# cbalint13/opencv-dlco

Hardware: AMD Instinct MI355X
Metric: pj-learn patch-pairs/sec (higher is better)
Workload: dtype f32; 1 GPU; pj-learn configs[1] Liberty-shaped, rank ~64: 500000 pair-rows x PR-dim 8192, batch 200+200 per GPU (global 200+200), mu=0.0025 gamma=0.5, fp32, rank 48 after 3893 steps; device= (gfx950:sramecc+:xnack-), burn_in_steps=300

## Files before the change

include/dlco.h:

```cpp
#ifndef DLCO_H
#define DLCO_H

#include <stddef.h>
#include <stdint.h>

#ifdef __cplusplus
extern "C" {
#endif

#define DLCO_OK            0
#define DLCO_ERR_INVALID  -2
#define DLCO_ERR_HIP      -3
#define DLCO_ERR_NODEVICE -4
#define DLCO_ERR_NOCONV   -5
#define DLCO_ERR_COMM     -6

typedef struct dlco_ctx dlco_ctx;

typedef struct dlco_cfg {
    int32_t  F;
    int32_t  N;
    int32_t  B;
    float    mu;
    float    gamma;
// ... 51 lines not shown
typedef int (*dlco_allgather_fn)(void *user, int32_t which, size_t bytes_per_rank);
int dlco_set_allgather(dlco_ctx *ctx, dlco_allgather_fn fn, void *user);
int dlco_comm_unique_id(void *out_id, size_t cap, const char *rccl_path);
int dlco_comm_init(dlco_ctx *ctx, const void *id, size_t id_bytes, const char *rccl_path);
int dlco_comm_init_host(dlco_ctx *ctx, const char *shm_name);
int dlco_comm_destroy(dlco_ctx *ctx);
int dlco_stream(dlco_ctx *ctx, void **stream);
int dlco_sync(dlco_ctx *ctx);

int dlco_get_batch(const dlco_ctx *ctx, int32_t *pos_rows, int32_t *neg_rows,
                   float *pos_dist, float *neg_dist, int32_t *rho, int32_t *kappa);

int dlco_get_t(const dlco_ctx *ctx, uint32_t *t);
int dlco_get_W(dlco_ctx *ctx, float *W_host , int32_t *r);
int dlco_get_A(dlco_ctx *ctx, float *A_host );
int dlco_get_dfavg(dlco_ctx *ctx, float *dfavg_host );
int dlco_set_state(dlco_ctx *ctx, uint32_t t, const float *dfavg_host, const float *W_host, int32_t r);

int dlco_validate(dlco_ctx *ctx, float *loss_val, float *regul, int32_t *rank);

int dlco_stats(dlco_ctx *ctx, const float *W_host, int32_t r, int32_t *dim, float *fpr95, double *auc);

int dlco_project_sqdist(dlco_ctx *ctx, const int32_t *row_ids_host, int32_t n,
                        const float *W_host, int32_t r, float *out_host);
int dlco_viol_counts(dlco_ctx *ctx, const float *pd_host, const float *nd_host, int32_t B,
                     int32_t *rho_host, int32_t *kappa_host);
int dlco_grad_rda(dlco_ctx *ctx, const int32_t *pos_rows_host, const int32_t *neg_rows_host,
                  const int32_t *rho_host, const int32_t *kappa_host, int32_t B,
                  float alpha, float beta, const float *dfavg_in_host, float *dfavg_out_host);
int dlco_psd_project(dlco_ctx *ctx, const float *dfavg_host, uint32_t t,
                     float *W_host, int32_t *r, float *A_host );
int dlco_sym_product(dlco_ctx *ctx, const float *X_host, int32_t rows, const float *G_host, int32_t mode,
                     float *out_host);
int dlco_hinge_sum(dlco_ctx *ctx, const float *pos_host, int32_t n_pos,
                   const float *neg_host, int32_t n_neg, double *out);
int dlco_roc_stats(dlco_ctx *ctx, const float *dist_host, const uint8_t *labels_host, int32_t n,
                   float *fpr95, double *auc);

typedef struct dlco_log_entry {
    uint32_t t;
    int32_t  is_best;
    int32_t  saved;
    float    loss_val, regul, obj, obj_best;
    int32_t  rank, rank_best;
    int32_t  dim;
    double   auc, auc_best;
    float    fpr95, fpr95_best;
    double   vtime;
    int32_t  nonconv;
    int32_t  reserved;
} dlco_log_entry;
int dlco_log_step(dlco_ctx *ctx, dlco_log_entry *out);
int dlco_get_saved(dlco_ctx *ctx, float *W_host, int32_t *r, float *A_host);

int dlco_profile_enable(dlco_ctx *ctx, int32_t on);
int dlco_profile_read(dlco_ctx *ctx, const char *kernel, int64_t *launches, double *total_ms);
int dlco_counters(const dlco_ctx *ctx, int64_t out[8]);
int dlco_eig_stats(const dlco_ctx *ctx, int64_t *iters, int64_t *product_rows, int64_t *jacobi_sweeps,
                   int32_t *block_rows);

typedef struct dlco_pr_ctx dlco_pr_ctx;
const char *dlco_pr_last_error(const dlco_pr_ctx *ctx);
int dlco_pr_create(dlco_pr_ctx **out, int32_t F, int32_t N, float mu, float gamma, uint64_t seed, int32_t device);
void dlco_pr_destroy(dlco_pr_ctx *ctx);
int dlco_pr_device_name(const dlco_pr_ctx *ctx, char *buf, size_t cap, int *cc_major, int *cc_minor);
int dlco_pr_set_data(dlco_pr_ctx *ctx, const float *dists_host, const uint8_t *labels_host);
// ... 98 lines not shown
```

opencv-dlco_amd/__init__.py:

```python
import ctypes as C
import os
import subprocess

import numpy as np

_HERE = os.path.dirname(os.path.abspath(__file__))
LIB_PATH = os.path.join(_HERE, "libdlco.so")
HEADER_PATH = os.path.join(os.path.dirname(_HERE), "include", "dlco.h")

OK, ERR_INVALID, ERR_HIP, ERR_NODEVICE, ERR_NOCONV, ERR_COMM = 0, -2, -3, -4, -5, -6
BUF_DIST, BUF_GRAD, BUF_DFAVG, BUF_W, BUF_GATHER, BUF_DATA = 1, 2, 3, 4, 5, 6
ALLGATHER_FN = C.CFUNCTYPE(C.c_int, C.c_void_p, C.c_int32, C.c_size_t)
DETECT_THRESHOLD = 100 * 100 * 256 * 256


class DlcoError(RuntimeError):
    def __init__(self, code, msg):
        super().__init__("libdlco error %d: %s" % (code, msg))
        self.code = code


class Cfg(C.Structure):
    _fields_ = [
        ("F", C.c_int32), ("N", C.c_int32), ("B", C.c_int32),
        ("mu", C.c_float), ("gamma", C.c_float),
        ("seed", C.c_uint64),
        ("device", C.c_int32), ("rank", C.c_int32), ("world", C.c_int32),
        ("eig_tol", C.c_float), ("eig_guard", C.c_int32), ("eig_max_iter", C.c_int32),
        ("shard", C.c_int32), ("strict_conv", C.c_int32), ("grad_bf16", C.c_int32),
        ("reserved", C.c_int32 * 5),
    ]


class LogEntry(C.Structure):
    _fields_ = [
        ("t", C.c_uint32), ("is_best", C.c_int32), ("saved", C.c_int32),
        ("loss_val", C.c_float), ("regul", C.c_float), ("obj", C.c_float), ("obj_best", C.c_float),
        ("rank", C.c_int32), ("rank_best", C.c_int32), ("dim", C.c_int32),
        ("auc", C.c_double), ("auc_best", C.c_double),
        ("fpr95", C.c_float), ("fpr95_best", C.c_float),
        ("vtime", C.c_double),
        ("nonconv", C.c_int32), ("reserved", C.c_int32),
    ]


def build(verbose=False):
    cmd = ["make", "-C", os.path.join(_HERE, "csrc"), "-j8"]
    if not verbose:
        cmd.insert(1, "-s")
    subprocess.check_call(cmd)


_lib = None
f32p, i32p, u8p = C.POINTER(C.c_float), C.POINTER(C.c_int32), C.POINTER(C.c_uint8)


def load():
    global _lib
    if _lib is not None:
        return _lib
    if not os.path.exists(LIB_PATH):
        raise DlcoError(ERR_NODEVICE, "%s is missing: run __graft_entry__.build() (no CPU fallback exists)" % LIB_PATH)
    L = C.CDLL(LIB_PATH)
    vp = C.c_void_p
    L.dlco_version.restype = C.c_char_p
    L.dlco_last_error.restype = C.c_char_p
    L.dlco_last_error.argtypes = [vp]
    L.dlco_cfg_default.argtypes = [C.POINTER(Cfg)]
    L.dlco_cfg_default.restype = None
    L.dlco_ctx_create.argtypes = [C.POINTER(vp), C.POINTER(Cfg)]
    L.dlco_ctx_destroy.argtypes = [vp]
    L.dlco_ctx_destroy.restype = None
    L.dlco_device_name.argtypes = [vp, C.c_char_p, C.c_size_t, C.POINTER(C.c_int), C.POINTER(C.c_int)]
    L.dlco_set_data.argtypes = [vp, f32p, u8p]
    L.dlco_set_data_device.argtypes = [vp, vp, u8p]
    L.dlco_set_data_shared.argtypes = [vp, vp]
    L.dlco_device_width.argtypes = [vp]
    L.dlco_set_pairs.argtypes = [vp, f32p, C.c_int32, i32p]
    L.dlco_synth_data.argtypes = [vp, f32p, C.c_int32, C.c_uint64, C.c_float, C.c_float, C.c_float, C.c_float]
    L.dlco_get_rows.argtypes = [vp, C.c_int32, C.c_int32, f32p]
    L.dlco_get_index.argtypes = [vp, i32p, i32p, i32p, i32p, i32p, i32p]
    for name in ("dlco_step", "dlco_step_begin", "dlco_step_grad", "dlco_step_finish", "dlco_sync"):
        getattr(L, name).argtypes = [vp]
    L.dlco_steps.argtypes = [vp, C.c_int32]
    L.dlco_dev_buffer.argtypes = [vp, C.c_int32, C.POINTER(vp), C.POINTER(C.c_size_t)]
    L.dlco_bind_buffer.argtypes = [vp, C.c_int32, vp, C.c_size_t]
    L.dlco_stream.argtypes = [vp, C.POINTER(vp)]
    L.dlco_set_allgather.argtypes = [vp, ALLGATHER_FN, vp]
    L.dlco_comm_unique_id.argtypes = [vp, C.c_size_t, C.c_char_p]
    L.dlco_comm_init.argtypes = [vp, vp, C.c_size_t, C.c_char_p]
    L.dlco_comm_destroy.argtypes = [vp]
    L.dlco_get_batch.argtypes = [vp, i32p, i32p, f32p, f32p, i32p, i32p]
    L.dlco_get_t.argtypes = [vp, C.POINTER(C.c_uint32)]
    L.dlco_get_W.argtypes = [vp, f32p, i32p]
    L.dlco_get_A.argtypes = [vp, f32p]
    L.dlco_get_dfavg.argtypes = [vp, f32p]
    L.dlco_set_state.argtypes = [vp, C.c_uint32, f32p, f32p, C.c_int32]
    L.dlco_validate.argtypes = [vp, f32p, f32p, i32p]
    L.dlco_stats.argtypes = [vp, f32p, C.c_int32, i32p, f32p, C.POINTER(C.c_double)]
    L.dlco_project_sqdist.argtypes = [vp, i32p, C.c_int32, f32p, C.c_int32, f32p]
    L.dlco_viol_counts.argtypes = [vp, f32p, f32p, C.c_int32, i32p, i32p]
    L.dlco_grad_rda.argtypes = [vp, i32p, i32p, i32p, i32p, C.c_int32, C.c_float, C.c_float, f32p, f32p]
    L.dlco_psd_project.argtypes = [vp, f32p, C.c_uint32, f32p, i32p, f32p]
    L.dlco_hinge_sum.argtypes = [vp, f32p, C.c_int32, f32p, C.c_int32, C.POINTER(C.c_double)]
    L.dlco_sym_product.argtypes = [vp, f32p, C.c_int32, f32p, C.c_int32, f32p]
    L.dlco_roc_stats.argtypes = [vp, f32p, u8p, C.c_int32, f32p, C.POINTER(C.c_double)]
    L.dlco_log_step.argtypes = [vp, C.POINTER(LogEntry)]
    L.dlco_get_saved.argtypes = [vp, f32p, i32p, f32p]
    L.dlco_profile_enable.argtypes = [vp, C.c_int32]
    L.dlco_profile_read.argtypes = [vp, C.c_char_p, C.POINTER(C.c_int64), C.POINTER(C.c_double)]
    L.dlco_eig_stats.argtypes = [vp, C.POINTER(C.c_int64), C.POINTER(C.c_int64), C.POINTER(C.c_int64), i32p]
    L.dlco_counters.argtypes = [vp, C.POINTER(C.c_int64)]
    i64 = C.c_int64
    L.dlco_set_pairs_device.argtypes = [vp, vp, C.c_int32, i32p]
    L.dlco_desc_last_error.restype = C.c_char_p
    L.dlco_desc_last_error.argtypes = [vp]
    L.dlco_desc_create.argtypes = [C.POINTER(vp), C.c_float, C.c_int32, C.c_int32, C.c_int32]
    L.dlco_desc_destroy.argtypes = [vp]
    L.dlco_desc_destroy.restype = None
    L.dlco_desc_select_filters.argtypes = [f32p, C.c_int32, C.c_int32, f32p, C.c_int32, f32p, C.POINTER(C.c_int32)]
    L.dlco_desc_set_filters.argtypes = [vp, f32p, C.c_int32]
    L.dlco_desc_size.argtypes = [vp]
    L.dlco_desc_size.restype = C.c_int32
    L.dlco_desc_transform.argtypes = [vp, u8p, f32p]
    L.dlco_desc_compute.argtypes = [vp, u8p, i64, f32p]
    L.dlco_desc_compute_device.argtypes = [vp, u8p, i64, vp, i64]
    L.dlco_desc_pair_dists.argtypes = [vp, u8p, i64, i32p, i64, f32p, u8p]
    L.dlco_desc_full_dists.argtypes = [vp, u8p, i64, i32p, i64, f32p, u8p]
    L.dlco_desc_set_projection.argtypes = [vp, f32p, C.c_int32, C.c_int32]
    L.dlco_desc_projected_size.argtypes = [vp]
    L.dlco_desc_projected_size.restype = C.c_int32
    L.dlco_desc_describe.argtypes = [vp, u8p, i64, f32p]
    L.dlco_desc_describe_device.argtypes = [vp, u8p, i64, vp, i64]
    L.dlco_desc_set_image.argtypes = [vp, u8p, C.c_int32, C.c_int32, i64]
    L.dlco_desc_set_image_device.argtypes = [vp, vp, C.c_int32, C.c_int32, i64]
    L.dlco_desc_extract_patches.argtypes = [vp, f32p, i64, C.c_float, C.c_int32, u8p, u8p]
    L.dlco_desc_describe_keypoints.argtypes = [vp, f32p, i64, C.c_float, C.c_int32, f32p, u8p]
    L.dlco_desc_describe_keypoints_device.argtypes = [vp, f32p, i64, C.c_float, C.c_int32, vp, i64, u8p]
# ... 277 lines not shown
    def project_sqdist(self, row_ids, W):
        ids, w = _i32(row_ids), _f32(W)
        out = np.empty(ids.size, np.float32)
        self._ck(self.L.dlco_project_sqdist(self.h, _p(ids, i32p), ids.size, _p(w, f32p), w.shape[0] if w.size else 0, _p(out, f32p)))
        return out

    def viol_counts(self, pd, nd):
        pd, nd = _f32(pd), _f32(nd)
        rho, kap = np.empty(pd.size, np.int32), np.empty(pd.size, np.int32)
        self._ck(self.L.dlco_viol_counts(self.h, _p(pd, f32p), _p(nd, f32p), pd.size, _p(rho, i32p), _p(kap, i32p)))
        return rho, kap

    def grad_rda(self, pos_rows, neg_rows, rho, kappa, alpha, beta, dfavg_in=None):
        pr, nr, rho, kap = _i32(pos_rows), _i32(neg_rows), _i32(rho), _i32(kappa)
        d = None if dfavg_in is None else _f32(dfavg_in)
        out = np.empty((self.F, self.F), np.float32)
        self._ck(self.L.dlco_grad_rda(self.h, _p(pr, i32p), _p(nr, i32p), _p(rho, i32p), _p(kap, i32p), pr.size, alpha, beta, _p(d, f32p), _p(out, f32p)))
        return out

    def psd_project(self, dfavg, t, want_A=True):
        d = _f32(dfavg)
        W = np.empty((self.F, self.F), np.float32)
        A = np.empty((self.F, self.F), np.float32) if want_A else None
        r = C.c_int32()
        self._ck(self.L.dlco_psd_project(self.h, _p(d, f32p), t, _p(W, f32p), C.byref(r), _p(A, f32p)))
        return W[:r.value].copy(), A

    def sym_product(self, X, G, mode=0):
        x, g = _f32(X), _f32(G)
        out = np.empty_like(x)
        self._ck(self.L.dlco_sym_product(self.h, _p(x, f32p), x.shape[0], _p(g, f32p), mode, _p(out, f32p)))
        return out

    def hinge_sum(self, pos, neg):
        p, n = _f32(pos), _f32(neg)
        out = C.c_double()
        self._ck(self.L.dlco_hinge_sum(self.h, _p(p, f32p), p.size, _p(n, f32p), n.size, C.byref(out)))
        return out.value

    def roc_stats(self, dist, labels):
        d, l = _f32(dist), np.ascontiguousarray(labels, np.uint8).ravel()
        f, a = C.c_float(), C.c_double()
        self._ck(self.L.dlco_roc_stats(self.h, _p(d, f32p), _p(l, u8p), d.size, C.byref(f), C.byref(a)))
        return f.value, a.value

    def profile_enable(self, on=True):
        self._ck(self.L.dlco_profile_enable(self.h, int(on)))

    def profile_read(self, kernel="grad_syrk"):
        n, ms = C.c_int64(), C.c_double()
        self._ck(self.L.dlco_profile_read(self.h, kernel.encode(), C.byref(n), C.byref(ms)))
        return n.value, ms.value

    def counters(self):
        out = (C.c_int64 * 8)()
        self._ck(self.L.dlco_counters(self.h, out))
        return dict(steps=out[0], active_rows=out[1], nonconverged=out[2], jacobi_barrier_timeouts=out[3],
                    rank_update_passes=out[4], rank_update_check=out[5] * 1e-9, locked_passes=out[6], locked_rows=out[7])

    def eig_stats(self):
        a, b, c_, d = C.c_int64(), C.c_int64(), C.c_int64(), C.c_int32()
        self._ck(self.L.dlco_eig_stats(self.h, C.byref(a), C.byref(b), C.byref(c_), C.byref(d)))
        return dict(iters=a.value, product_rows=b.value, jacobi_sweeps=c_.value, block_rows=d.value)


class PrContext:
# ... 411 lines not shown
```

opencv-dlco_amd/csrc/dlco_api.cpp:

```cpp
#include "../../include/dlco.h"

#include "dlco_internal.hpp"
#include "eig_tracker.hpp"
#include "pair_index.hpp"
#include "rccl_comm.hpp"
#include "host_comm.hpp"

#include <algorithm>
#include <cfloat>
#include <chrono>
#include <cmath>
#include <cstring>

using namespace dlco;

static thread_local std::string g_last_error;

namespace {
struct EnvSwitch { const char *name, *purpose; };
const EnvSwitch kEnvSwitches[] = {
    {"DLCO_SYRK_FP32", "gradient SYRK as the k-ordered fp32 MFMA chain (syrk_rda_kernel8) instead of split-bf16 planes"},
    {"DLCO_NO_PACKED", "full F x F dual average where the packed upper-tile form would apply"},
    {"DLCO_FORCE_SHARD", "column-sharded layout (cfg.shard) on a single rank: the multi-GPU path on one GPU"},
    {"DLCO_NO_RANK_UPDATE", "first filter term from a product with the dual average, not from the step's rank update"},
// ... 1109 lines not shown
            ok = skinny_product_sym(X.p, F, rows, Gp.p, F, 1.0f, out.p, F, nullptr, 0.f, nullptr, 0.f, hi.p, lo.p, slab.p, c->stream,
                                    mode == 4 ? lo2.p : nullptr);
            sync(c);
        } else if (mode == 1 || mode == 2) {
            DevBuf<char> hi, lo, lo2;
            hi.alloc(bf16x2_plane_bytes(rows, F)); lo.alloc(bf16x2_plane_bytes(rows, F));
            if (mode == 2) lo2.alloc(bf16x2_plane_bytes(rows, F));
            DevBuf<float> slab;
            slab.alloc(bf16x2_slab_floats(rows, F));
            ok = skinny_product_bf16x2(X.p, F, rows, G.p, F, F, F, 1.0f, out.p, F, nullptr, 0.f, nullptr, 0.f, hi.p, lo.p, slab.p,
                                       c->stream, 0, mode == 2 ? lo2.p : nullptr);
            sync(c);
        } else {
            GemmArgs g;
            g.M = rows; g.N = F; g.K = F;
            g.A.p = X.p; g.A.ld = F; g.A.kmajor = false;
            g.B.p = G.p; g.B.ld = F; g.B.kmajor = true;
            g.C = out.p; g.ldc = F;
            const int bm = rows <= 64 ? 64 : 128;
            const long tiles = (long)((rows + bm - 1) / bm) * ((F + 127) / 128);
            g.split_k = split_k_slices(tiles, 1024, F, 256);
            DevBuf<float> slab;
            slab.alloc(gemm_slab_floats(rows, F, g.split_k));
            g.slab = slab.p;
            gemm_f32(g, c->stream);
            sync(c);
            ok = true;
        }
        DLCO_CHECK(ok, DLCO_ERR_INVALID, "dlco_sym_product: shape not supported by this mode");
        d2h_rows(c, out_host, out.p, (size_t)rows);
    });
}

int dlco_hinge_sum(dlco_ctx *c, const float *pos_host, int32_t n_pos, const float *neg_host, int32_t n_neg, double *out)
{
    if (!c || !out || n_pos < 0 || n_neg < 0) return DLCO_ERR_INVALID;
    return guarded(c, [&] {
        DLCO_HIP(hipSetDevice(c->cfg.device));
        *out = 0.0;
        if (n_pos == 0) return;
        DevBuf<float> p, n, rows;
        p.alloc(n_pos); n.alloc(std::max(n_neg, 1)); rows.alloc(n_pos);
        h2d(c, p.p, pos_host, (size_t)n_pos * sizeof(float));
        if (n_neg) h2d(c, n.p, neg_host, (size_t)n_neg * sizeof(float));
        hinge_rows(p.p, n_pos, n.p, n_neg, rows.p, c->stream);
        sum_f32_to_f64(rows.p, n_pos, c->dscal.p, c->stream);
        d2h(c, out, c->dscal.p, sizeof(double));
    });
}

int dlco_roc_stats(dlco_ctx *c, const float *dist_host, const uint8_t *labels_host, int32_t n, float *fpr95, double *auc)
{
    if (!c || !dist_host || !labels_host || !fpr95 || !auc || n < 1) return DLCO_ERR_INVALID;
    return guarded(c, [&] {
        DLCO_HIP(hipSetDevice(c->cfg.device));
        DevBuf<float> d; DevBuf<uint8_t> l;
        d.alloc(n); l.alloc(n);
        h2d(c, d.p, dist_host, (size_t)n * sizeof(float));
        h2d(c, l.p, labels_host, (size_t)n);
        RocWork *w = roc_work_create(n);
        try { roc_stats(w, d.p, l.p, n, fpr95, auc, c->stream); } catch (...) { roc_work_destroy(w); throw; }
        roc_work_destroy(w);
    });
}

int dlco_log_step(dlco_ctx *c, dlco_log_entry *out)
// ... 110 lines not shown
```

opencv-dlco_amd/csrc/dlco_internal.hpp:

```cpp
#pragma once

#include "../../include/dlco.h"
#include "match_slices.hpp"

#include <hip/hip_runtime.h>

#include <algorithm>
#include <climits>
#include <cstdint>
#include <cstdio>
#include <cstdlib>
#include <cstring>
#include <functional>
#include <mutex>
#include <utility>
#include <stdexcept>
#include <string>
#include <type_traits>
#include <vector>

namespace patch_rules { struct Frame; }

namespace dlco {

// ... 121 lines not shown
        r.used = 0;
    }
    void drain_all() { for (int i = 0; i < PROF_SLOTS; i++) drain(i); }
    void reset() { drain_all(); for (auto &r : rec) { r.ms = 0.0; r.n = 0; } }
};

struct GemmOperand {
    const float *p = nullptr;
    long ld = 0;
    bool kmajor = false;
    const int32_t *row_ids = nullptr;
    const int32_t *row_ids2 = nullptr;
    const float *row_scale = nullptr;
};

struct GemmArgs {
    int M = 0, N = 0, K = 0;
    GemmOperand A, B;
    float *C = nullptr;
    long ldc = 0;
    float alpha = 1.0f, beta = 0.0f;
    const float *E1 = nullptr;
    float b1 = 0.0f;
    const float *E2 = nullptr;
    float b2 = 0.0f;
    const int *k_dev = nullptr;
    int split_k = 1;
    float *slab = nullptr;
    bool upper_only = false;
    const float *B2 = nullptr;
    float *C2 = nullptr;
    bool small_m_tiles = false;
    bool small_n_tiles = false;
};

void gemm_f32(const GemmArgs &a, hipStream_t s);
size_t bf16x2_plane_bytes(int M, int K);
size_t bf16x2_slab_floats(int M, int N, int ksplit = 0);
void split_planes_bf16(const float *X, long ldx, int M, int K, void *hi, void *lo, void *lo2, hipStream_t s);
bool skinny_product_bf16x2(const float *X, long ldx, int M, const float *G, long ldg, int N, int K, float alpha, float *C,
                           long ldc, const float *E1, float b1, const float *E2, float b2, void *plane_hi, void *plane_lo,
                           float *slab, hipStream_t s, int ksplit = 0, void *plane_lo2 = nullptr, bool g_tiled = false);
size_t project_rows_plane_bytes(int K);
bool project_rows_sqdist(const float *W, long ldw, int r, const float *D, long ldd, int F, const int32_t *ids, const int32_t *ids2,
                         long row0, int nrows, float *dist, void *plane_hi, void *plane_lo, void *plane_lo2, bool bf16, hipStream_t s);
bool project_rows_slab(const float *W, long ldw, int r, const float *D, long ldd, int F, const int32_t *ids, const int32_t *ids2,
                       int nrows, int ksplit, float *slab, long ldn, void *plane_hi, void *plane_lo, void *plane_lo2, bool bf16,
                       hipStream_t s);
struct RankCoeffJob {
    const float *proj = nullptr;
    long ldp = 0;
    int nw = 0, m = 0, MT = 0;
    const float *wscale = nullptr;
    const int32_t *slot = nullptr;
    void *frag = nullptr;
};
void syrk_mirror_upper(float *C, long ldc, int F, hipStream_t s);
size_t syrk_planes_bytes(int kmax, int F);
bool syrk_rda_f32(const float *D, long ldd, const int32_t *ids, const int32_t *ids2, const float *w, const int *k_dev,
                  int kmax, int F, float alpha, float beta, float *C, long ldc, hipStream_t s, int slab_col0 = 0,
                  int slab_cols = 0, bool bf16 = false, bool packed = false, void *planes_ws = nullptr,
                  const RankCoeffJob *coeff_job = nullptr);
int syrk_planes_mode(bool bf16);
size_t rank_coeff_bytes(int m, int kmax);
bool rank_first_term(const float *Y, const float *Q, long ld, int m, int F, float ay, float aq, float ac, float *out,
                     const float *proj, long ldp, int nw, const float *wscale, const int32_t *slot, const float *w,
                     const int *k_dev, int kmax, const void *planes, void *coeff_ws, void *plane_hi, void *plane_lo, hipStream_t s,
                     bool coeff_ready = false, int planes_mode = 3);
size_t syrk_packed_floats(int F);
// ... 115 lines not shown
```

opencv-dlco_amd/csrc/kernels_gemm.hip:

```cpp
#include "dlco_internal.hpp"

namespace dlco {

typedef float f32x16 __attribute__((ext_vector_type(16)));
typedef float f32x4 __attribute__((ext_vector_type(4)));

namespace {

constexpr int BK = 16;
constexpr int PAD = 4;
constexpr int NT = 256;

struct OperandDev {
    const float *p;
    long ld;
    const int32_t *row_ids;
    const float *row_scale;
    int vec_ok;
    const int32_t *row_ids2;
};

__device__ __forceinline__ f32x4 load4(const float *src, int pos, int limit, int vec_ok)
{
    f32x4 v = {0.f, 0.f, 0.f, 0.f};
    if (vec_ok && pos + 3 < limit) {
        v = *reinterpret_cast<const f32x4 *>(src);
    } else {
        v[0] = src[0];
        if (pos + 1 < limit) v[1] = src[1];
        if (pos + 2 < limit) v[2] = src[2];
        if (pos + 3 < limit) v[3] = src[3];
    }
    return v;
}

struct GemmDev {
    int M, N, K;
    OperandDev A, B;
    float *C;
    long ldc;
    float alpha, beta, b1, b2;
    const float *E1, *E2;
    const int *k_dev;
    int k_chunk;
// ... 7 lines not shown
__device__ __forceinline__ void load_tile(const OperandDev &op, int t0, int tmax, int k0, int kend,
                                          f32x4 (&regs)[BT / 64])
{
    const int tid = threadIdx.x;
#pragma unroll
    for (int u = 0; u < BT / 64; u++) {
        const int f = tid + NT * u;
        f32x4 v = {0.f, 0.f, 0.f, 0.f};
        if (KM) {
            const int row = f / (BT / 4), c4 = f % (BT / 4);
            const int k = k0 + row, col = t0 + c4 * 4;
            if (k < kend && col < tmax) {
                const long mr = op.row_ids ? (long)op.row_ids[k] : (long)k;
                v = load4(op.p + mr * op.ld + col, col, tmax, op.vec_ok);
                if (op.row_ids2) v -= load4(op.p + (long)op.row_ids2[k] * op.ld + col, col, tmax, op.vec_ok);
                if (op.row_scale) {
                    const float sc = op.row_scale[k];
                    v *= sc;
                }
            }
        } else {
            const int row = f / (BK / 4), kq = f % (BK / 4);
            const int t = t0 + row, k = k0 + kq * 4;
            if (t < tmax && k < kend) {
                const long mr = op.row_ids ? (long)op.row_ids[t] : (long)t;
                v = load4(op.p + mr * op.ld + k, k, kend, op.vec_ok);
                if (op.row_ids2) v -= load4(op.p + (long)op.row_ids2[t] * op.ld + k, k, kend, op.vec_ok);
            }
        }
        regs[u] = v;
    }
}

template <int BT, bool KM>
__device__ __forceinline__ void store_tile(float (*lds)[BT + PAD], const f32x4 (&regs)[BT / 64])
{
    const int tid = threadIdx.x;
#pragma unroll
    for (int u = 0; u < BT / 64; u++) {
        const int f = tid + NT * u;
        if (KM) {
            const int row = f / (BT / 4), c4 = f % (BT / 4);
            *reinterpret_cast<f32x4 *>(&lds[row][c4 * 4]) = regs[u];
        } else {
            const int row = f / (BK / 4), kq = f % (BK / 4);
            lds[kq * 4 + 0][row] = regs[u][0];
            lds[kq * 4 + 1][row] = regs[u][1];
            lds[kq * 4 + 2][row] = regs[u][2];
            lds[kq * 4 + 3][row] = regs[u][3];
        }
    }
}

template <int WM, int WN, bool A_KM, bool B_KM>
__global__ __launch_bounds__(NT) void gemm_kernel(GemmDev g)
{
    constexpr int BM = 64 * WM, BN = 64 * WN;
    __shared__ __attribute__((aligned(16))) float As[2][BK][BM + PAD];
    __shared__ __attribute__((aligned(16))) float Bs[2][BK][BN + PAD];

    const int bi = blockIdx.y, bj = blockIdx.x;
    if (g.upper_only && bj * BN + BN <= bi * BM) return;
    const int i0 = bi * BM, j0 = bj * BN;
    const int lane = threadIdx.x & 63, wave = threadIdx.x >> 6;
    const int wm = wave >> 1, wn = wave & 1;

    int kz = blockIdx.z;
    if (g.B2) {
        if (kz == 1) { g.B.p = g.B2; g.C = g.C2; }
        kz = 0;
    }
    int kbeg = kz * g.k_chunk;
    int kend = min(g.K, kbeg + g.k_chunk);
    if (g.k_dev) kend = min(kend, *g.k_dev);

    f32x16 acc[WM][WN];
#pragma unroll
    for (int a = 0; a < WM; a++)
#pragma unroll
        for (int b = 0; b < WN; b++)
#pragma unroll
            for (int r = 0; r < 16; r++) acc[a][b][r] = 0.f;

    const int nk = kend > kbeg ? (kend - kbeg + BK - 1) / BK : 0;
    f32x4 ra[BM / 64], rb[BN / 64];
    if (nk > 0) {
        load_tile<BM, A_KM>(g.A, i0, g.M, kbeg, kend, ra);
        load_tile<BN, B_KM>(g.B, j0, g.N, kbeg, kend, rb);
        store_tile<BM, A_KM>(As[0], ra);
        store_tile<BN, B_KM>(Bs[0], rb);
    }
    __syncthreads();
    for (int kt = 0; kt < nk; kt++) {
        const int buf = kt & 1;
        if (kt + 1 < nk) {
            load_tile<BM, A_KM>(g.A, i0, g.M, kbeg + (kt + 1) * BK, kend, ra);
            load_tile<BN, B_KM>(g.B, j0, g.N, kbeg + (kt + 1) * BK, kend, rb);
        }
        const int lr = lane & 31, lk = lane >> 5;
#pragma unroll
        for (int kk = 0; kk < BK / 2; kk++) {
            float af[WM], bf[WN];
#pragma unroll
            for (int a = 0; a < WM; a++) af[a] = As[buf][2 * kk + lk][wm * 32 * WM + a * 32 + lr];
#pragma unroll
            for (int b = 0; b < WN; b++) bf[b] = Bs[buf][2 * kk + lk][wn * 32 * WN + b * 32 + lr];
#pragma unroll
            for (int a = 0; a < WM; a++)
#pragma unroll
                for (int b = 0; b < WN; b++)
                    acc[a][b] = __builtin_amdgcn_mfma_f32_32x32x2f32(af[a], bf[b], acc[a][b], 0, 0, 0);
        }
        if (kt + 1 < nk) {
            store_tile<BM, A_KM>(As[buf ^ 1], ra);
            store_tile<BN, B_KM>(Bs[buf ^ 1], rb);
        }
        __syncthreads();
    }

    const int lc = lane & 31, lh = lane >> 5;
#pragma unroll
    for (int a = 0; a < WM; a++)
#pragma unroll
        for (int b = 0; b < WN; b++)
#pragma unroll
            for (int r = 0; r < 16; r++) {
                const int i = i0 + wm * 32 * WM + a * 32 + (r & 3) + 8 * (r >> 2) + 4 * lh;
                const int j = j0 + wn * 32 * WN + b * 32 + lc;
                if (i >= g.M || j >= g.N) continue;
                if (g.slab) {
                    g.slab[((long)blockIdx.z * g.M + i) * g.N + j] = acc[a][b][r];
                    continue;
                }
                if (g.upper_only && j < i) continue;
                const long idx = (long)i * g.ldc + j;
                float o = g.alpha * acc[a][b][r];
                if (g.beta != 0.f) o += g.beta * g.C[idx];
                if (g.E1) o += g.b1 * g.E1[idx];
                if (g.E2) o += g.b2 * g.E2[idx];
                g.C[idx] = o;
                if (g.upper_only && j > i) g.C[(long)j * g.ldc + i] = o;
            }
}

__global__ void splitk_reduce_kernel(const float *slab, int split, int M, int N, float *C, long ldc, float alpha,
                                     float beta, const float *E1, float b1, const float *E2, float b2)
{
    const long total = (long)M * N;
    const int zl = threadIdx.x & 15;
    for (long e = ((long)blockIdx.x * blockDim.x + threadIdx.x) >> 4; e < total; e += ((long)gridDim.x * blockDim.x) >> 4) {
// ... 3 lines not shown
        s += __int_as_float(__builtin_amdgcn_update_dpp(0, __float_as_int(s), 0xB1, 0xF, 0xF, true));
        s += __int_as_float(__builtin_amdgcn_update_dpp(0, __float_as_int(s), 0x4E, 0xF, 0xF, true));
        s += __int_as_float(__builtin_amdgcn_update_dpp(0, __float_as_int(s), 0x141, 0xF, 0xF, true));
        s += __int_as_float(__builtin_amdgcn_update_dpp(0, __float_as_int(s), 0x140, 0xF, 0xF, true));
        if (zl != 0) continue;
        const long idx = (long)i * ldc + j;
        float o = alpha * s;
        if (beta != 0.f) o += beta * C[idx];
        if (E1) o += b1 * E1[idx];
        if (E2) o += b2 * E2[idx];
        C[idx] = o;
    }
}

__global__ __launch_bounds__(256) void splitk_reduce_wide_kernel(const float *slab, int split, int M, int N, float *C,
                                                                 long ldc, float alpha, float beta, const float *E1,
                                                                 float b1, const float *E2, float b2)
{
    const long total = (long)M * N, q = N >> 2;
    for (long e = (long)blockIdx.x * blockDim.x + threadIdx.x; e < (long)M * q; e += (long)gridDim.x * blockDim.x) {
        const int i = (int)(e / q), j = (int)(e % q) * 4;
        const float *p = slab + (long)i * N + j;
        f32x4 s = *reinterpret_cast<const f32x4 *>(p);
        for (int z = 1; z < split; z++) s += *reinterpret_cast<const f32x4 *>(p + (long)z * total);
        const long idx = (long)i * ldc + j;
        f32x4 o = alpha * s;
        if (beta != 0.f) o += beta * *reinterpret_cast<const f32x4 *>(C + idx);
        if (E1) o += b1 * *reinterpret_cast<const f32x4 *>(E1 + idx);
        if (E2) o += b2 * *reinterpret_cast<const f32x4 *>(E2 + idx);
        *reinterpret_cast<f32x4 *>(C + idx) = o;
    }
}

template <int WM, int WN>
void launch(const GemmDev &g, bool akm, bool bkm, dim3 grid, hipStream_t s)
{
    if (akm && bkm) hipLaunchKernelGGL((gemm_kernel<WM, WN, true, true>), grid, dim3(NT), 0, s, g);
    else if (akm && !bkm) hipLaunchKernelGGL((gemm_kernel<WM, WN, true, false>), grid, dim3(NT), 0, s, g);
    else if (!akm && bkm) hipLaunchKernelGGL((gemm_kernel<WM, WN, false, true>), grid, dim3(NT), 0, s, g);
    else hipLaunchKernelGGL((gemm_kernel<WM, WN, false, false>), grid, dim3(NT), 0, s, g);
}

inline int vec_ok(const GemmOperand &o) { return (o.ld % 4 == 0) && ((reinterpret_cast<uintptr_t>(o.p) & 15) == 0); }

}

size_t gemm_slab_floats(int M, int N, int split_k) { return split_k > 1 ? (size_t)split_k * M * N : 0; }

void splitk_reduce_f32(const float *slab, int split, int M, int N, float *C, long ldc, float alpha, float beta,
                       const float *E1, float b1, const float *E2, float b2, hipStream_t s)
{
    const long total = (long)M * N;
    auto al16 = [](const void *p) { return (reinterpret_cast<uintptr_t>(p) & 15) == 0; };
    if (split <= 32 && total >= 65536 && N % 4 == 0 && ldc % 4 == 0 && al16(slab) && al16(C) && (!E1 || al16(E1)) &&
        (!E2 || al16(E2))) {
        long blocks = (total / 4 + 255) / 256;
        if (blocks > 4096) blocks = 4096;
        hipLaunchKernelGGL(splitk_reduce_wide_kernel, dim3((unsigned)blocks), dim3(256), 0, s, slab, split, M, N, C, ldc, alpha,
                           beta, E1, b1, E2, b2);
        DLCO_HIP(hipGetLastError());
        return;
    }
    long blocks = (total * 16 + 255) / 256;
    if (blocks > 8192) blocks = 8192;
    hipLaunchKernelGGL(splitk_reduce_kernel, dim3((unsigned)blocks), dim3(256), 0, s, slab, split, M, N, C, ldc, alpha, beta,
                       E1, b1, E2, b2);
    DLCO_HIP(hipGetLastError());
}

void gemm_f32(const GemmArgs &a, hipStream_t s)
{
    if (a.M <= 0 || a.N <= 0) return;
    DLCO_CHECK(a.A.p && a.B.p && a.C, -2, "gemm_f32: null operand");
    DLCO_CHECK(!(a.upper_only && (a.M != a.N || a.split_k > 1)), -2, "gemm_f32: upper_only needs M==N, split_k==1");
    GemmDev g;
    g.M = a.M; g.N = a.N; g.K = a.K;
    g.A = {a.A.p, a.A.ld, a.A.row_ids, a.A.kmajor ? a.A.row_scale : nullptr, vec_ok(a.A), a.A.row_ids2};
    g.B = {a.B.p, a.B.ld, a.B.row_ids, a.B.kmajor ? a.B.row_scale : nullptr, vec_ok(a.B), a.B.row_ids2};
    g.C = a.C; g.ldc = a.ldc;
    g.alpha = a.alpha; g.beta = a.beta; g.E1 = a.E1; g.b1 = a.b1; g.E2 = a.E2; g.b2 = a.b2;
    g.k_dev = a.k_dev;
    g.upper_only = a.upper_only ? 1 : 0;
    int split = a.split_k < 1 ? 1 : a.split_k;
    int chunk = (a.K + split - 1) / split;
    chunk = ((chunk + BK - 1) / BK) * BK;
    if (chunk < BK) chunk = BK;
    split = a.K > 0 ? (a.K + chunk - 1) / chunk : 1;
    g.k_chunk = chunk;
    g.slab = nullptr;
    if (split > 1) {
        DLCO_CHECK(a.slab != nullptr, -2, "gemm_f32: split_k > 1 needs a slab workspace");
        g.slab = a.slab;
    }
    g.B2 = a.B2; g.C2 = a.C2;
    if (a.B2) {
        DLCO_CHECK(a.C2 && split == 1 && !a.upper_only, -2, "gemm_f32: a twin product needs C2 and no K split");
        split = 2;
    }
    bool small_m = a.M <= 64 || a.small_m_tiles, small_n = a.N <= 64 || a.small_n_tiles;
    auto n_wg = [&](bool sm, bool sn) {
        return (long)((a.M + (sm ? 63 : 127)) / (sm ? 64 : 128)) * ((a.N + (sn ? 63 : 127)) / (sn ? 64 : 128)) * split;
    };
    if (!a.upper_only) {
        if (!small_m && n_wg(small_m, small_n) < 256) small_m = true;
        if (!small_n && n_wg(small_m, small_n) < 256) small_n = true;
    }
    if (small_m && small_n) {
        dim3 grid((a.N + 63) / 64, (a.M + 63) / 64, split);
        launch<1, 1>(g, a.A.kmajor, a.B.kmajor, grid, s);
    } else if (small_m) {
        dim3 grid((a.N + 127) / 128, (a.M + 63) / 64, split);
        launch<1, 2>(g, a.A.kmajor, a.B.kmajor, grid, s);
    } else if (small_n) {
        dim3 grid((a.N + 63) / 64, (a.M + 127) / 128, split);
        launch<2, 1>(g, a.A.kmajor, a.B.kmajor, grid, s);
    } else {
        dim3 grid((a.N + 127) / 128, (a.M + 127) / 128, split);
        launch<2, 2>(g, a.A.kmajor, a.B.kmajor, grid, s);
    }
    DLCO_HIP(hipGetLastError());
    if (split > 1 && !a.B2)
        splitk_reduce_f32(a.slab, split, a.M, a.N, a.C, a.ldc, a.alpha, a.beta, a.E1, a.b1, a.E2, a.b2, s);
}

}
```

Before: 719,800 pair-rows/s.

## Add register ring prefetch of depth four to small-tile GEMM kernels

Result: faster. 734,200 pair-rows/s, median of 6 (+2.0%).

```diff
diff --git a/include/dlco.h b/include/dlco.h
--- a/include/dlco.h
+++ b/include/dlco.h
@@ -107,6 +107,23 @@
                      float *W_host, int32_t *r, float *A_host );
 int dlco_sym_product(dlco_ctx *ctx, const float *X_host, int32_t rows, const float *G_host, int32_t mode,
                      float *out_host);
+typedef struct dlco_gemm_operand {
+    const float   *host;
+    int32_t        rows, ld;
+    int32_t        kmajor;
+    const int32_t *row_ids, *row_ids2;
+    const float   *row_scale;
+} dlco_gemm_operand;
+typedef struct dlco_gemm_probe_args {
+    int32_t M, N, K;
+    dlco_gemm_operand A, B;
+    const float *B2_host;
+    int32_t split_k, k_dev, small_m_tiles, small_n_tiles, depth, reps;
+    float   alpha, beta, b1, b2;
+    const float *E1_host, *E2_host;
+} dlco_gemm_probe_args;
+int dlco_gemm_probe(dlco_ctx *ctx, const dlco_gemm_probe_args *args, float *C_host, float *C2_host, int32_t *depth_used,
+                    double *us_per_launch);
 int dlco_hinge_sum(dlco_ctx *ctx, const float *pos_host, int32_t n_pos,
                    const float *neg_host, int32_t n_neg, double *out);
 int dlco_roc_stats(dlco_ctx *ctx, const float *dist_host, const uint8_t *labels_host, int32_t n,
diff --git a/opencv-dlco_amd/__init__.py b/opencv-dlco_amd/__init__.py
--- a/opencv-dlco_amd/__init__.py
+++ b/opencv-dlco_amd/__init__.py
@@ -41,6 +41,25 @@
         ("fpr95", C.c_float), ("fpr95_best", C.c_float),
         ("vtime", C.c_double),
         ("nonconv", C.c_int32), ("reserved", C.c_int32),
+    ]
+
+
+class GemmOperand(C.Structure):
+    _fields_ = [
+        ("host", C.POINTER(C.c_float)), ("rows", C.c_int32), ("ld", C.c_int32), ("kmajor", C.c_int32),
+        ("row_ids", C.POINTER(C.c_int32)), ("row_ids2", C.POINTER(C.c_int32)), ("row_scale", C.POINTER(C.c_float)),
+    ]
+
+
+class GemmProbeArgs(C.Structure):
+    _fields_ = [
+        ("M", C.c_int32), ("N", C.c_int32), ("K", C.c_int32),
+        ("A", GemmOperand), ("B", GemmOperand),
+        ("B2_host", C.POINTER(C.c_float)),
+        ("split_k", C.c_int32), ("k_dev", C.c_int32), ("small_m_tiles", C.c_int32), ("small_n_tiles", C.c_int32),
+        ("depth", C.c_int32), ("reps", C.c_int32),
+        ("alpha", C.c_float), ("beta", C.c_float), ("b1", C.c_float), ("b2", C.c_float),
+        ("E1_host", C.POINTER(C.c_float)), ("E2_host", C.POINTER(C.c_float)),
     ]
 
 
@@ -104,6 +123,7 @@
     L.dlco_psd_project.argtypes = [vp, f32p, C.c_uint32, f32p, i32p, f32p]
     L.dlco_hinge_sum.argtypes = [vp, f32p, C.c_int32, f32p, C.c_int32, C.POINTER(C.c_double)]
     L.dlco_sym_product.argtypes = [vp, f32p, C.c_int32, f32p, C.c_int32, f32p]
+    L.dlco_gemm_probe.argtypes = [vp, C.POINTER(GemmProbeArgs), f32p, f32p, i32p, C.POINTER(C.c_double)]
     L.dlco_roc_stats.argtypes = [vp, f32p, u8p, C.c_int32, f32p, C.POINTER(C.c_double)]
     L.dlco_log_step.argtypes = [vp, C.POINTER(LogEntry)]
     L.dlco_get_saved.argtypes = [vp, f32p, i32p, f32p]
@@ -447,6 +467,38 @@
         self._ck(self.L.dlco_sym_product(self.h, _p(x, f32p), x.shape[0], _p(g, f32p), mode, _p(out, f32p)))
         return out
 
+    def gemm_probe(self, A, B, M, N, K, a_kmajor=False, b_kmajor=False, a_ids=None, a_ids2=None, a_scale=None, b_ids=None,
+                   b_ids2=None, b_scale=None, B2=None, split_k=1, k_dev=-1, small_m_tiles=False, small_n_tiles=False, depth=0,
+                   alpha=1.0, beta=0.0, C_in=None, E1=None, b1=0.0, E2=None, b2=0.0, reps=0):
+        keep = []
+
+        def operand(x, kmajor, ids, ids2, scale):
+            x = _f32(x)
+            assert x.ndim == 2
+            ids, ids2 = (None if i is None else _i32(i) for i in (ids, ids2))
+            scale = None if scale is None else _f32(scale)
+            keep.extend([x, ids, ids2, scale])
+            return GemmOperand(_p(x, f32p), x.shape[0], x.shape[1], int(kmajor), _p(ids, i32p), _p(ids2, i32p), _p(scale, f32p)), x
+
+        a = GemmProbeArgs()
+        a.M, a.N, a.K = M, N, K
+        a.A, _ = operand(A, a_kmajor, a_ids, a_ids2, a_scale)
+        a.B, b = operand(B, b_kmajor, b_ids, b_ids2, b_scale)
+        twin = None if B2 is None else _f32(B2)
+        assert twin is None or twin.shape == b.shape
+        e1, e2 = (None if e is None else _f32(e) for e in (E1, E2))
+        assert all(e is None or e.shape == (M, N) for e in (e1, e2))
+        a.B2_host, a.E1_host, a.E2_host = _p(twin, f32p), _p(e1, f32p), _p(e2, f32p)
+        a.split_k, a.k_dev, a.depth, a.reps = split_k, k_dev, depth, reps
+        a.small_m_tiles, a.small_n_tiles = int(small_m_tiles), int(small_n_tiles)
+        a.alpha, a.beta, a.b1, a.b2 = alpha, beta, b1, b2
+        out = np.zeros((M, N), np.float32) if C_in is None else np.array(C_in, dtype=np.float32, order="C")
+        assert out.shape == (M, N)
+        out2 = None if twin is None else out.copy()
+        used, us = C.c_int32(), C.c_double()
+        self._ck(self.L.dlco_gemm_probe(self.h, C.byref(a), _p(out, f32p), _p(out2, f32p), C.byref(used), C.byref(us)))
+        return dict(C=out, C2=out2, depth=used.value, us=us.value if reps else None)
+
     def hinge_sum(self, pos, neg):
         p, n = _f32(pos), _f32(neg)
         out = C.c_double()
diff --git a/opencv-dlco_amd/csrc/dlco_api.cpp b/opencv-dlco_amd/csrc/dlco_api.cpp
--- a/opencv-dlco_amd/csrc/dlco_api.cpp
+++ b/opencv-dlco_amd/csrc/dlco_api.cpp
@@ -1165,6 +1165,79 @@
     });
 }
 
+int dlco_gemm_probe(dlco_ctx *c, const dlco_gemm_probe_args *a, float *C_host, float *C2_host, int32_t *depth_used,
+                    double *us_per_launch)
+{
+    if (!c || !a || !C_host || a->M < 1 || a->N < 1 || a->K < 1 || a->split_k < 1 || a->reps < 0 || a->k_dev > a->K) return DLCO_ERR_INVALID;
+    if ((a->B2_host != nullptr) != (C2_host != nullptr)) return DLCO_ERR_INVALID;
+    return guarded(c, [&] {
+        DLCO_HIP(hipSetDevice(c->cfg.device));
+        auto check = [&](const dlco_gemm_operand &o, int t) {
+            const int along = o.kmajor ? t : a->K, ids = o.kmajor ? a->K : t;
+            DLCO_CHECK(o.host && o.rows >= 1 && o.ld >= along, DLCO_ERR_INVALID, "dlco_gemm_probe: operand smaller than the product");
+            DLCO_CHECK(!o.row_ids2 || o.row_ids, DLCO_ERR_INVALID, "dlco_gemm_probe: row_ids2 without row_ids");
+            DLCO_CHECK(!o.row_scale || o.kmajor, DLCO_ERR_INVALID, "dlco_gemm_probe: row_scale needs a k-major operand");
+            DLCO_CHECK(o.row_ids || o.rows >= ids, DLCO_ERR_INVALID, "dlco_gemm_probe: operand has too few rows");
+            for (const int32_t *id : {o.row_ids, o.row_ids2})
+                for (int x = 0; id && x < ids; x++)
+                    DLCO_CHECK(id[x] >= 0 && id[x] < o.rows, DLCO_ERR_INVALID, "dlco_gemm_probe: row id out of range");
+        };
+        check(a->A, a->M);
+        check(a->B, a->N);
+        struct Dev { DevBuf<float> p, scale; DevBuf<int32_t> ids, ids2; };
+        auto upload = [&](const dlco_gemm_operand &o, int t, const float *host, Dev &d, GemmOperand &g) {
+            const int ids = o.kmajor ? a->K : t;
+            d.p.alloc((size_t)o.rows * o.ld);
+            h2d(c, d.p.p, host, (size_t)o.rows * o.ld * sizeof(float));
+            g.p = d.p.p; g.ld = o.ld; g.kmajor = o.kmajor != 0;
+            if (o.row_ids) { d.ids.alloc(ids); h2d(c, d.ids.p, o.row_ids, (size_t)ids * sizeof(int32_t)); g.row_ids = d.ids.p; }
+            if (o.row_ids2) { d.ids2.alloc(ids); h2d(c, d.ids2.p, o.row_ids2, (size_t)ids * sizeof(int32_t)); g.row_ids2 = d.ids2.p; }
+            if (o.row_scale) { d.scale.alloc(a->K); h2d(c, d.scale.p, o.row_scale, (size_t)a->K * sizeof(float)); g.row_scale = d.scale.p; }
+        };
+        const size_t mn = (size_t)a->M * a->N;
+        Dev dA, dB, dB2;
+        DevBuf<float> C, C2, E1, E2, slab;
+        DevBuf<int> kdev;
+        GemmArgs g;
+        GemmOperand twin;
+        g.M = a->M; g.N = a->N; g.K = a->K;
+        upload(a->A, a->M, a->A.host, dA, g.A);
+        upload(a->B, a->N, a->B.host, dB, g.B);
+        if (a->B2_host) { upload(a->B, a->N, a->B2_host, dB2, twin); g.B2 = twin.p; C2.alloc(mn); g.C2 = C2.p; }
+        C.alloc(mn); g.C = C.p; g.ldc = a->N;
+        g.alpha = a->alpha; g.beta = a->beta; g.b1 = a->b1; g.b2 = a->b2;
+        if (a->E1_host) { E1.alloc(mn); h2d(c, E1.p, a->E1_host, mn * sizeof(float)); g.E1 = E1.p; }
+        if (a->E2_host) { E2.alloc(mn); h2d(c, E2.p, a->E2_host, mn * sizeof(float)); g.E2 = E2.p; }
+        if (a->k_dev >= 0) { const int k = a->k_dev; kdev.alloc(1); h2d(c, kdev.p, &k, sizeof(int)); g.k_dev = kdev.p; }
+        g.split_k = a->split_k;
+        slab.alloc(gemm_slab_floats(a->M, a->N, a->split_k)); g.slab = slab.p;
+        g.small_m_tiles = a->small_m_tiles != 0; g.small_n_tiles = a->small_n_tiles != 0;
+        g.depth = a->depth;
+        int used = 0;
+        g.depth_used = &used;
+        if (a->reps > 0) {
+            hipEvent_t e0, e1;
+            DLCO_HIP(hipEventCreate(&e0)); DLCO_HIP(hipEventCreate(&e1));
+            for (int i = 0; i < 3; i++) gemm_f32(g, c->stream);
+            DLCO_HIP(hipEventRecord(e0, c->stream));
+            for (int i = 0; i < a->reps; i++) gemm_f32(g, c->stream);
+            DLCO_HIP(hipEventRecord(e1, c->stream));
+            sync(c);
+            float ms = 0.f;
+            DLCO_HIP(hipEventElapsedTime(&ms, e0, e1));
+            (void)hipEventDestroy(e0); (void)hipEventDestroy(e1);
+            if (us_per_launch) *us_per_launch = 1e3 * ms / a->reps;
+        }
+        h2d(c, C.p, C_host, mn * sizeof(float));
+        if (C2_host) h2d(c, C2.p, C2_host, mn * sizeof(float));
+        gemm_f32(g, c->stream);
+        sync(c);
+        d2h(c, C_host, C.p, mn * sizeof(float));
+        if (C2_host) d2h(c, C2_host, C2.p, mn * sizeof(float));
+        if (depth_used) *depth_used = used;
+    });
+}
+
 int dlco_hinge_sum(dlco_ctx *c, const float *pos_host, int32_t n_pos, const float *neg_host, int32_t n_neg, double *out)
 {
     if (!c || !out || n_pos < 0 || n_neg < 0) return DLCO_ERR_INVALID;
diff --git a/opencv-dlco_amd/csrc/dlco_internal.hpp b/opencv-dlco_amd/csrc/dlco_internal.hpp
--- a/opencv-dlco_amd/csrc/dlco_internal.hpp
+++ b/opencv-dlco_amd/csrc/dlco_internal.hpp
@@ -177,9 +177,12 @@
     float *C2 = nullptr;
     bool small_m_tiles = false;
     bool small_n_tiles = false;
+    int depth = 0;
+    int *depth_used = nullptr;
 };
 
 void gemm_f32(const GemmArgs &a, hipStream_t s);
+int gemm_ring_depth();
 size_t bf16x2_plane_bytes(int M, int K);
 size_t bf16x2_slab_floats(int M, int N, int ksplit = 0);
 void split_planes_bf16(const float *X, long ldx, int M, int K, void *hi, void *lo, void *lo2, hipStream_t s);
diff --git a/opencv-dlco_amd/csrc/kernels_gemm.hip b/opencv-dlco_amd/csrc/kernels_gemm.hip
--- a/opencv-dlco_amd/csrc/kernels_gemm.hip
+++ b/opencv-dlco_amd/csrc/kernels_gemm.hip
@@ -10,6 +10,11 @@
 constexpr int BK = 16;
 constexpr int PAD = 4;
 constexpr int NT = 256;
+#ifndef DLCO_GEMM_DEPTH
+#define DLCO_GEMM_DEPTH 4
+#endif
+constexpr int RING_DEPTH = DLCO_GEMM_DEPTH;
+static_assert(RING_DEPTH == 2 || RING_DEPTH == 4 || RING_DEPTH == 8, "ring depth: 2, 4 or 8");
 
 struct OperandDev {
     const float *p;
@@ -83,6 +88,64 @@
     }
 }
 
+
+template <int BT>
+struct TileRows {
+    const float *r[BT / 64];
+};
+
+template <int BT, bool KM>
+__device__ __forceinline__ void tile_rows(const OperandDev &op, int t0, int tmax, TileRows<BT> &rows)
+{
+#pragma unroll
+    for (int u = 0; u < BT / 64; u++) {
+        rows.r[u] = op.p;
+        if (KM) continue;
+        const int t = min(t0 + (int)(threadIdx.x + NT * u) / (BK / 4), tmax - 1);
+        rows.r[u] = op.p + (op.row_ids ? (long)op.row_ids[t] : (long)t) * op.ld;
+    }
+}
+
+template <int BT, bool KM>
+__device__ __forceinline__ void fetch_plain(const OperandDev &op, const TileRows<BT> &rows, int t0, int tmax, int k0, int kend, int K,
+                                            f32x4 (&regs)[BT / 64])
+{
+    const int tid = threadIdx.x;
+#pragma unroll
+    for (int u = 0; u < BT / 64; u++) {
+        const int f = tid + NT * u;
+        if (KM) {
+            const int row = f / (BT / 4), c4 = f % (BT / 4);
+            regs[u] = *reinterpret_cast<const f32x4 *>(op.p + (long)min(k0 + row, kend - 1) * op.ld + min(t0 + c4 * 4, tmax - 4));
+        } else {
+            const int kq = f % (BK / 4);
+            regs[u] = *reinterpret_cast<const f32x4 *>(rows.r[u] + min(k0 + kq * 4, K - 4));
+        }
+    }
+}
+
+template <int BT, bool KM>
+__device__ __forceinline__ void zero_beyond(int t0, int tmax, int k0, int kend, f32x4 (&regs)[BT / 64])
+{
+    const int tid = threadIdx.x;
+#pragma unroll
+    for (int u = 0; u < BT / 64; u++) {
+        const int f = tid + NT * u;
+        int live;
+        if (KM) {
+            const int row = f / (BT / 4), c4 = f % (BT / 4);
+            live = (k0 + row < kend && t0 + c4 * 4 < tmax) ? 4 : 0;
+        } else {
+            const int row = f / (BK / 4), kq = f % (BK / 4);
+            live = t0 + row < tmax ? kend - (k0 + kq * 4) : 0;
+        }
+        regs[u][0] = live > 0 ? regs[u][0] : 0.f;
+        regs[u][1] = live > 1 ? regs[u][1] : 0.f;
+        regs[u][2] = live > 2 ? regs[u][2] : 0.f;
+        regs[u][3] = live > 3 ? regs[u][3] : 0.f;
+    }
+}
+
 template <int BT, bool KM>
 __device__ __forceinline__ void store_tile(float (*lds)[BT + PAD], const f32x4 (&regs)[BT / 64])
 {
@@ -103,7 +166,7 @@
     }
 }
 
-template <int WM, int WN, bool A_KM, bool B_KM>
+template <int WM, int WN, bool A_KM, bool B_KM, int DEPTH>
 __global__ __launch_bounds__(NT) void gemm_kernel(GemmDev g)
 {
     constexpr int BM = 64 * WM, BN = 64 * WN;
@@ -121,7 +184,7 @@
         if (kz == 1) { g.B.p = g.B2; g.C = g.C2; }
         kz = 0;
     }
-    int kbeg = kz * g.k_chunk;
+    const int kbeg = kz * g.k_chunk;
     int kend = min(g.K, kbeg + g.k_chunk);
     if (g.k_dev) kend = min(kend, *g.k_dev);
 
@@ -134,21 +197,35 @@
             for (int r = 0; r < 16; r++) acc[a][b][r] = 0.f;
 
     const int nk = kend > kbeg ? (kend - kbeg + BK - 1) / BK : 0;
-    f32x4 ra[BM / 64], rb[BN / 64];
     if (nk > 0) {
-        load_tile<BM, A_KM>(g.A, i0, g.M, kbeg, kend, ra);
-        load_tile<BN, B_KM>(g.B, j0, g.N, kbeg, kend, rb);
-        store_tile<BM, A_KM>(As[0], ra);
-        store_tile<BN, B_KM>(Bs[0], rb);
-    }
-    __syncthreads();
-    for (int kt = 0; kt < nk; kt++) {
-        const int buf = kt & 1;
-        if (kt + 1 < nk) {
-            load_tile<BM, A_KM>(g.A, i0, g.M, kbeg + (kt + 1) * BK, kend, ra);
-            load_tile<BN, B_KM>(g.B, j0, g.N, kbeg + (kt + 1) * BK, kend, rb);
-        }
-        const int lr = lane & 31, lk = lane >> 5;
+    TileRows<BM> rows_a;
+    TileRows<BN> rows_b;
+    if (DEPTH > 1) {
+        tile_rows<BM, A_KM>(g.A, i0, g.M, rows_a);
+        tile_rows<BN, B_KM>(g.B, j0, g.N, rows_b);
+    }
+    struct Slot { f32x4 a[BM / 64], b[BN / 64]; };
+    Slot ring[DEPTH];
+    auto request = [&](int p, Slot &s) {
+        if (DEPTH > 1) {
+            fetch_plain<BM, A_KM>(g.A, rows_a, i0, g.M, kbeg + p * BK, kend, g.K, s.a);
+            fetch_plain<BN, B_KM>(g.B, rows_b, j0, g.N, kbeg + p * BK, kend, g.K, s.b);
+        } else {
+            load_tile<BM, A_KM>(g.A, i0, g.M, kbeg + p * BK, kend, s.a);
+            load_tile<BN, B_KM>(g.B, j0, g.N, kbeg + p * BK, kend, s.b);
+        }
+    };
+    auto commit = [&](int buf, int p, const Slot &s) {
+        Slot t = s;
+        if (DEPTH > 1) {
+            zero_beyond<BM, A_KM>(i0, g.M, kbeg + p * BK, kend, t.a);
+            zero_beyond<BN, B_KM>(j0, g.N, kbeg + p * BK, kend, t.b);
+        }
+        store_tile<BM, A_KM>(As[buf], t.a);
+        store_tile<BN, B_KM>(Bs[buf], t.b);
+    };
+    const int lr = lane & 31, lk = lane >> 5;
+    auto multiply = [&](int buf) {
 #pragma unroll
         for (int kk = 0; kk < BK / 2; kk++) {
             float af[WM], bf[WN];
@@ -162,11 +239,30 @@
                 for (int b = 0; b < WN; b++)
                     acc[a][b] = __builtin_amdgcn_mfma_f32_32x32x2f32(af[a], bf[b], acc[a][b], 0, 0, 0);
         }
-        if (kt + 1 < nk) {
-            store_tile<BM, A_KM>(As[buf ^ 1], ra);
-            store_tile<BN, B_KM>(Bs[buf ^ 1], rb);
-        }
-        __syncthreads();
+    };
+
+#pragma unroll
+    for (int d = 0; d < DEPTH; d++) request(d, ring[d]);
+    commit(0, 0, ring[0]);
+    __syncthreads();
+    int kt = 0;
+    for (; kt + DEPTH <= nk; kt += DEPTH) {
+#pragma unroll
+        for (int d = 0; d < DEPTH; d++) {
+            request(kt + d + DEPTH, ring[d]);
+            multiply((kt + d) & 1);
+            commit(((kt + d) & 1) ^ 1, kt + d + 1, ring[(d + 1) % DEPTH]);
+            __syncthreads();
+        }
+    }
+#pragma unroll
+    for (int d = 0; d + 1 < DEPTH; d++) {
+        if (kt + d < nk) {
+            multiply((kt + d) & 1);
+            commit(((kt + d) & 1) ^ 1, kt + d + 1, ring[d + 1]);
+            __syncthreads();
+        }
+    }
     }
 
     const int lc = lane & 31, lh = lane >> 5;
@@ -236,16 +332,29 @@
     }
 }
 
+template <int WM, int WN, int DEPTH>
+void launch(const GemmDev &g, bool akm, bool bkm, dim3 grid, hipStream_t s)
+{
+    if (akm && bkm) hipLaunchKernelGGL((gemm_kernel<WM, WN, true, true, DEPTH>), grid, dim3(NT), 0, s, g);
+    else if (akm && !bkm) hipLaunchKernelGGL((gemm_kernel<WM, WN, true, false, DEPTH>), grid, dim3(NT), 0, s, g);
+    else if (!akm && bkm) hipLaunchKernelGGL((gemm_kernel<WM, WN, false, true, DEPTH>), grid, dim3(NT), 0, s, g);
+    else hipLaunchKernelGGL((gemm_kernel<WM, WN, false, false, DEPTH>), grid, dim3(NT), 0, s, g);
+}
+
 template <int WM, int WN>
-void launch(const GemmDev &g, bool akm, bool bkm, dim3 grid, hipStream_t s)
-{
-    if (akm && bkm) hipLaunchKernelGGL((gemm_kernel<WM, WN, true, true>), grid, dim3(NT), 0, s, g);
-    else if (akm && !bkm) hipLaunchKernelGGL((gemm_kernel<WM, WN, true, false>), grid, dim3(NT), 0, s, g);
-    else if (!akm && bkm) hipLaunchKernelGGL((gemm_kernel<WM, WN, false, true>), grid, dim3(NT), 0, s, g);
-    else hipLaunchKernelGGL((gemm_kernel<WM, WN, false, false>), grid, dim3(NT), 0, s, g);
+void launch_small(const GemmDev &g, bool akm, bool bkm, dim3 grid, bool ring, hipStream_t s)
+{
+    if (ring) launch<WM, WN, RING_DEPTH>(g, akm, bkm, grid, s);
+    else launch<WM, WN, 1>(g, akm, bkm, grid, s);
 }
 
 inline int vec_ok(const GemmOperand &o) { return (o.ld % 4 == 0) && ((reinterpret_cast<uintptr_t>(o.p) & 15) == 0); }
+
+inline bool plain_operand(const GemmOperand &o, int t, int K)
+{
+    if (!vec_ok(o) || o.row_ids2 || (o.kmajor && (o.row_scale || o.row_ids))) return false;
+    return (o.kmajor ? t : K) % 4 == 0;
+}
 
 }
 
@@ -272,9 +381,12 @@
     DLCO_HIP(hipGetLastError());
 }
 
+int gemm_ring_depth() { return RING_DEPTH; }
+
 void gemm_f32(const GemmArgs &a, hipStream_t s)
 {
     if (a.M <= 0 || a.N <= 0) return;
+    DLCO_CHECK(a.depth == 0 || a.depth == 1, -2, "gemm_f32: depth is 0 (the library's choice) or 1");
     DLCO_CHECK(a.A.p && a.B.p && a.C, -2, "gemm_f32: null operand");
     DLCO_CHECK(!(a.upper_only && (a.M != a.N || a.split_k > 1)), -2, "gemm_f32: upper_only needs M==N, split_k==1");
     GemmDev g;
@@ -309,18 +421,20 @@
         if (!small_m && n_wg(small_m, small_n) < 256) small_m = true;
         if (!small_n && n_wg(small_m, small_n) < 256) small_n = true;
     }
+    const bool ring = a.depth != 1 && plain_operand(a.A, a.M, a.K) && plain_operand(a.B, a.N, a.K);
+    if (a.depth_used) *a.depth_used = ring && (small_m || small_n) ? RING_DEPTH : 1;
     if (small_m && small_n) {
         dim3 grid((a.N + 63) / 64, (a.M + 63) / 64, split);
-        launch<1, 1>(g, a.A.kmajor, a.B.kmajor, grid, s);
+        launch_small<1, 1>(g, a.A.kmajor, a.B.kmajor, grid, ring, s);
     } else if (small_m) {
         dim3 grid((a.N + 127) / 128, (a.M + 63) / 64, split);
-        launch<1, 2>(g, a.A.kmajor, a.B.kmajor, grid, s);
+        launch_small<1, 2>(g, a.A.kmajor, a.B.kmajor, grid, ring, s);
     } else if (small_n) {
         dim3 grid((a.N + 63) / 64, (a.M + 127) / 128, split);
-        launch<2, 1>(g, a.A.kmajor, a.B.kmajor, grid, s);
+        launch_small<2, 1>(g, a.A.kmajor, a.B.kmajor, grid, ring, s);
     } else {
         dim3 grid((a.N + 127) / 128, (a.M + 127) / 128, split);
-        launch<2, 2>(g, a.A.kmajor, a.B.kmajor, grid, s);
+        launch<2, 2, 1>(g, a.A.kmajor, a.B.kmajor, grid, s);
     }
     DLCO_HIP(hipGetLastError());
     if (split > 1 && !a.B2)
```
